# liuruiyang98/Jittor-MLP

Measured on AMD Instinct MI355X. Metric: images/sec fwd, 224^2 bs=256/GPU, Mixer-B/16, higher is better.
Workload: dtype bf16

## Files before the change

### jittor-mlp_amd/csrc/gen/t4emu.py

```python
import os
import struct
import sys

import numpy as np

sys.path.insert(0, os.path.dirname(os.path.abspath(__file__)))
import isa
import t4gen
from q4emu import from16, gelu_ref, to16

S_TOK, KPAD = 196, 224


def w2_slot_source():
    slot = np.arange(32)
    kk, h, e = slot >> 4, (slot >> 3) & 1, slot & 7
    return 16 * kk + 8 * (e >> 2) + 4 * h + (e & 3)


def pack(w1, b1, w2, b2, dt, dt2=None):
    T, S = w1.shape
    G = (T + 31) // 32
    w1p = np.zeros((G * 32, 256), np.uint16)
    w1p[:T, :S] = to16(w1, dt)
# ... 25 lines not shown
        q = f16(c[0] * u + c[1]).astype(np.float64)
        for k in range(2, 7):
            q = f16(q * u + c[k]).astype(np.float64)
        p = np.clip(f16(t * q + 0.5).astype(np.float64), 0.0, 1.0)
        return f16(h * p).astype(np.float64)


def plan(M, t_rows, G, grid, nimg):
    tpi = t_rows // 256
    nit = G + 2
    lead = nit & 1
    return dict(M=M, G=G, ldxt=KPAD, ldx=t_rows, ntiles=M // 256, tpi=tpi, tpi_magic=(((1 << 31) + tpi - 1) // tpi) & 0xFFFFFFFF,
                grid=grid, stat_ld=nimg * S_TOK * 2, nit=nit + lead, lead=lead, S=S_TOK)


class T4Emu(isa.Emu):
    def __init__(self, gen, mem, karg_addr, bid, **kw):
        asm = isa.Asm()
        asm.ins = list(gen.a.ins)
        super().__init__(asm, mem, lds_bytes=163840, nwaves=4, **kw)
        self.karg_addr, self.bid = karg_addr, bid

    def init(self, waves):
        for w in waves:
            w.s[0] = self.karg_addr & 0xFFFFFFFF
            w.s[1] = self.karg_addr >> 32
            w.s[2] = self.bid
            w.v[0] = (np.arange(64) + 64 * w.wid).astype(np.uint32)
            w.v[1:] = 0x7FC0BEEF
            w.a[:] = 0x7FC0BEEF
        self.lds[:] = 0xEE


def run_case(gen, nimg=1, t_rows=512, T=80, grid=1, seed=0, dma_mode="late", order=None, verbose=False):
    rng = np.random.default_rng(seed)
    dt = gen.dtype
    S = S_TOK
    M = nimg * t_rows
    xt = np.zeros((M, KPAD), np.uint16)
    xt[:, :S] = to16(rng.uniform(-1, 1, (M, S)), dt)
    w1 = rng.uniform(-1, 1, (T, S)) * 0.15
    b1 = rng.uniform(-1, 1, T).astype(np.float32)
    w2 = rng.uniform(-1, 1, (S, T)) * 0.2
    b2 = rng.uniform(-1, 1, S).astype(np.float32)
    x0 = to16(rng.uniform(-2, 2, (nimg * S, t_rows)), dt)
    ln = getattr(gen, "ln", False)
    if ln:
        gamma = rng.uniform(0.5, 1.5, t_rows).astype(np.float32)
        beta = rng.uniform(-0.5, 0.5, t_rows).astype(np.float32)
        xf = from16(x0, dt).astype(np.float64)
        mean = xf.mean(axis=1).astype(np.float32)
        rstd = (1.0 / np.sqrt(xf.var(axis=1) + 1e-5)).astype(np.float32)
        xn = ((xf - mean[:, None].astype(np.float64)) * rstd[:, None].astype(np.float64)) * gamma[None, :] + beta[None, :]
        xt[:, :S] = to16(xn.reshape(nimg, S, t_rows).transpose(0, 2, 1).reshape(M, S), dt)
    dt2 = "f16" if getattr(gen, "h2", False) else dt
    w1p, b1p, w2p, b2p, G = pack(w1, b1, w2, b2, dt, dt2)
    mem = isa.Mem()
    aXt, aW1, aW2, aB1, aB2 = mem.add(xt), mem.add(w1p), mem.add(w2p), mem.add(b1p), mem.add(b2p)
    aX = mem.add(x0, writable=True)
    nplanes = t_rows // 64
    stats = np.full((nplanes, nimg * S, 2), np.nan, np.float32)
    aSt = mem.add(stats, writable=True)
    pl = plan(M, t_rows, G, grid, nimg)
    ka = bytearray(t4gen.ARG_BYTES)
    for name, val in (("xt", aXt), ("w1", aW1), ("w2", aW2), ("b1", aB1), ("b2", aB2), ("x", aX), ("stats", aSt), ("prof", 0)):
        struct.pack_into("<Q", ka, t4gen.KA[name], val)
    for name, val in pl.items():
        struct.pack_into("<I", ka, t4gen.KA[name], val)
    if ln:
        for name, arr in (("ln_mean", mean), ("ln_rstd", rstd), ("gamma", gamma), ("beta", beta)):
            struct.pack_into("<Q", ka, t4gen.KA[name], mem.add(arr))
        struct.pack_into("<Q", ka, t4gen.KA["xt"], 0)
    karg = mem.add(np.frombuffer(bytes(ka), np.uint8))
    nins = 0
    for bid in range(grid):
        e = T4Emu(gen, mem, karg, bid, dma_mode=dma_mode, order=order)
        waves = e.run()
        nins += sum(w.nissued for w in waves)
    out = from16(mem.get(aX).view(np.uint16).reshape(nimg * S, t_rows), dt).astype(np.float64)
    X = from16(xt[:, :S], dt).astype(np.float64)
    W1 = from16(to16(w1, dt), dt).astype(np.float64)
    W2 = from16(to16(w2, dt2), dt2).astype(np.float64)
    hid = gelu_ref(X @ W1.T + b1[None, :].astype(np.float64))
    hid = from16(to16(hid, dt2), dt2).astype(np.float64)
    y = hid @ W2.T + b2[None, :].astype(np.float64)
    y = y.reshape(nimg, t_rows, S).transpose(0, 2, 1).reshape(nimg * S, t_rows)
    ref = from16(to16(y + from16(x0, dt).astype(np.float64), dt), dt).astype(np.float64)
    err = np.abs(out - ref)
    tol = (2.0 ** -7 * 2.0 if dt == "bf16" else 2.0 ** -10 * 1.5) * np.maximum(1.0, np.abs(ref))
    bad = ~(err <= tol)
    ok = not bad.any()
    if getattr(gen, "h2", False):
        pre = (X @ W1.T).astype(np.float32) + b1[None, :]
        y2 = h2_gelu_ref(pre) @ W2.T + b2[None, :].astype(np.float64)
        y2 = y2.reshape(nimg, t_rows, S).transpose(0, 2, 1).reshape(nimg * S, t_rows)
        ref2 = from16(to16(y2 + from16(x0, dt).astype(np.float64), dt), dt).astype(np.float64)
        d2 = np.abs(out - ref2)
        ulp = 2.0 ** (np.floor(np.log2(np.maximum(np.abs(ref2), 0.5))) - 7)
        frac = float((d2 > 0).mean())
        if verbose:
            print("  against the operation-by-operation restatement of the packed-f16 GELU: %.2f %% of the outputs differ, max %.2f ulp" %
                  (100 * frac, float((d2 / ulp).max())))
        if not ((d2 <= ulp).all() and frac < 0.03):
            print("  FAILED the restatement check: %.2f %% differ, max %.2f ulp" % (100 * frac, float((d2 / ulp).max())))
            ok = False
    if verbose or bad.any():
        print("case nimg=%d t_rows=%d T=%d (G=%d) grid=%d mode=%s: bad %d of %d, max err %.3g, instructions %d" %
              (nimg, t_rows, T, G, grid, dma_mode, bad.sum(), bad.size, np.nanmax(err) if np.isfinite(err).any() else float("nan"), nins))
        if bad.any():
            idx = np.argwhere(bad)
            print("  first bad (token row, channel):", idx[:8].tolist())
# ... 23 lines not shown
```

### jittor-mlp_amd/csrc/gen/t4gen.py

```python
import os
import sys

sys.path.insert(0, os.path.dirname(os.path.abspath(__file__)))
from isa import A, F, S, V, Asm, Neg, Reg, h2bits
from q4gen import GELU, GELU_FORM, GELU_H2, GELU_RAW, GELU_SIG, SQRT2, Alloc, h2_gelu_ops, h2b_gelu_ops, sig_gelu_ops

KA = dict(xt=0, w1=8, w2=16, b1=24, b2=32, x=40, stats=48, prof=56,
          M=64, G=68, ldxt=72, ldx=76, ntiles=80, tpi=84, tpi_magic=88, grid=92, stat_ld=96, nit=100, lead=104, S=108,
          ln_mean=112, ln_rstd=120, gamma=128, beta=136)
ARG_BYTES = 144
LN_WAVE = 2 * 8 * 272

W1_PITCH, W1_PIECES = 528, 17
W2_PITCH, W2_PIECES = 80, 18
W1_STAGE, W2_STAGE = W1_PIECES * 1024, W2_PIECES * 1024
W1_OFF, W2_OFF = 0, 2 * W1_STAGE
B1_OFF = W2_OFF + 2 * W2_STAGE
STG_PITCH = 272
STG_WAVE = 32 * STG_PITCH
STG_OFF = B1_OFF + 4096
STG_BUF = 4 * STG_WAVE
LDS_BYTES = STG_OFF + 2 * STG_BUF
W2_GROUP_BYTES = 224 * 64
W1_MAGIC, W2_MAGIC = 1986, 13108
assert all((o * W1_MAGIC) >> 20 == o // W1_PITCH for o in range(0, W1_STAGE, 16))
assert all((o * W2_MAGIC) >> 20 == o // W2_PITCH for o in range(0, W2_STAGE, 16))


class T4:
    NKS, NTB = 13, 7
    NXA = 8
    DEPTH = 3

    def __init__(self, dtype="bf16", stats=False, dbg=0, name=None, shape=0, ln=False, h2=False):
        assert not ln or shape
        self.ln = ln
        self.shape = shape
        self.dtype, self.stats, self.dbg = dtype, stats, dbg
        assert not h2 or dtype == "bf16"
        self.h2 = h2
        self.name = name or "t4_%s%s%s%s" % (dtype, "_h2" if h2 else "", "_st" if stats else "", ("", "_odd", "_even")[shape] + ("_ln" if ln else ""))
        self.mfma = "v_mfma_f32_32x32x16_bf16" if dtype == "bf16" else "v_mfma_f32_32x32x16_f16"
        self.mfma2 = "v_mfma_f32_32x32x16_f16" if h2 else self.mfma
        self.cvt = "v_cvt_pk_bf16_f32" if dtype == "bf16" else "v_cvt_pk_f16_f32"
        self.dot = "v_dot2c_f32_bf16" if dtype == "bf16" else "v_dot2c_f32_f16"
        self.raw = GELU_RAW[dtype]
        self.coefs = GELU[dtype][1]
        self.a = Asm()
        self.build()

    def regs(self):
        s = Alloc("s", 33, 100)
        v = Alloc("v", 1, 256)
        self.s_karg, self.s_bid, self.v_tid = S(0, 2), S(2), V(0)
        self.p = {k: S(4 + 2 * i, 2) for i, k in enumerate(["xt", "w1", "w2", "b1", "b2", "x", "stats", "prof"])}
        self.k = {k: S(20 + i) for i, k in enumerate(["M", "G", "ldxt", "ldx", "ntiles", "tpi", "tpi_magic", "grid", "stat_ld", "nit", "lead", "S"])}
        self.s_wave, self.s_tile, self.s_next, self.s_has = s("wave"), s("tile"), s("next"), s("has")
        self.s_g, self.s_cnt = s("g"), s("cnt")
        self.s_wv1k, self.s_w2x = s("wv1k"), s("w2x")
        self.s_w1src, self.s_w2src = s("w1src", 2, 2), s("w2src", 2, 2)
        self.s_xb = [s("xb%d" % rb, 2, 2) for rb in range(2)]
        self.s_ocur, self.s_lcur = s("ocur", 2, 2), s("lcur", 2, 2)
        self.s_scur = s("scur", 2, 2) if self.stats else None
        self.s_tok8 = s("tok8")
        self.s_r2 = s("r2")
        self.sig = GELU_FORM[self.dtype] == "sig" and not self.h2
        self.h2b = GELU_FORM[self.dtype] == "h2b" and not self.h2
        self.s_k0, self.s_k1 = (s("gk0"), s("gk1")) if (self.sig or self.h2b) else (None, None)
        self.s_hscale, self.s_hc6 = (s("hscale"), s("hc6")) if self.h2 else (None, None)
        self.s_mask = s("mask", 2, 2)
        self.s_t = [s("t%d" % i) for i in range(6)]
        self.s_t64 = s("t64", 2, 2)
        self.s_prof0 = s("prof0", 2, 2)
        self.s_prof1, self.s_epi = s("prof1", 2, 2), s("epi")
        self.s_ph = [s("ph%d" % i) for i in range(3)]
        if self.ln:
            self.s_lnp = s("lnp", 8, 4)
            self.s_lx, self.s_lmean, self.s_lrstd = s("lx", 2, 2), s("lmean", 2, 2), s("lrstd", 2, 2)
            self.s_l16 = s("l16")
        self.ns = s.next
        self.X = [[None] * self.NKS for _ in range(2)]
        na = 0
        for rb in range(2):
            for ks in range(self.NKS):
                if rb == 1 and ks >= self.NKS - self.NXA:
                    self.X[rb][ks] = A(224 + 4 * na, 4)
                    na += 1
                else:
                    self.X[rb][ks] = v("X%d_%d" % (rb, ks), 4, 2)
        self.Wf = [v("Wf%d" % b, 4, 2) for b in range(4)]
        self.b1 = v("b1", 16, 2)
        self.xg = [[v("xg%d_%d" % (par, rb), 16, 2) for rb in range(2)] for par in range(2)]
        self.h = [[[v("h%d_%d_%d" % (par, rb, kk), 4, 2) for kk in range(2)] for rb in range(2)] for par in range(2)]
        self.tmp = [[v("g%s%d" % (n, ch), 2, 2) for n in "tuq"] for ch in range(2)]
        flat = [r_[e] for grp_ in self.tmp for r_ in grp_ for e in range(2)]
        self.tmp_t, self.tmp_u, self.tmp_q = flat[0:4], flat[4:8], flat[8:12]
        self.v_c0 = v("c0")
        self.v_hc = [v("hc%d" % j) for j in range(1, 6)] if (self.h2 or self.h2b) else None
        self.v_hp = [v("hp%d" % j) for j in range(2)] if self.h2b else None
        self.v_nz = v("negzero") if self.h2b else None
        self.v_w1rd, self.v_w2rd, self.v_b1rd = v("w1rd"), v("w2rd"), v("b1rd")
        self.v_w1off = [v("w1off%d" % i) for i in range(5)]
        self.v_w2off = [v("w2off%d" % i) for i in range(5)]
        self.v_xoff = v("xoff")
        self.v_stw, self.v_strd, self.v_ooff = v("stw"), v("strd"), v("ooff")
        self.v_soff = v("soff") if self.stats else None
        self.v_b2 = [v("b2_%d" % tb) for tb in range(self.NTB)]
        self.nv = v.next
# ... 200 lines not shown
            self.wait_lds(rd[n])
            wf = self.Wf[n & 3]
            for rb in range(2):
                if kind == "w2":
                    mfma(self.D2(rb, tb), self.h[par][rb][x], wf, self.D2(rb, tb), op=self.mfma2)
                else:
                    mfma(self.xg[par][rb], wf, self.X[rb][x], self.b1 if x == 0 else self.xg[par][rb])
        while state["done"] < total:
            fill[state["done"]]()
            state["done"] += 1
        while xl:
            emit_xload()
        assert not dma
        a("s_add_i32", self.s_g, self.s_g, 1)
        a("v_add_u32", self.v_b1rd, 128, self.v_b1rd)

    def tile_xbase(self, tile):
        a, t, k = self.a, self.s_t, self.k
        a("s_lshl_b32", t[0], tile, 8)
        a("s_lshl_b32", t[1], self.s_wave, 6)
        a("s_add_u32", t[0], t[0], t[1])
        self.mul64(self.s_t64, t[0], k["ldxt"], 1)
        self.add64(self.s_xb[0], self.p["xt"], self.s_t64[0], self.s_t64[1])
        a("s_lshl_b32", t[0], k["ldxt"], 6)
        self.add64(self.s_xb[1], self.s_xb[0], t[0])

    def x_loads(self):
        if self.dbg & 32:
            return
        for rb in range(2):
            for ks in range(self.NKS):
                self.vload("global_load_dwordx4", self.X[rb][ks], self.v_xoff, self.s_xb[rb], offset=32 * ks)

    def ln_loader(self, tile):
        a, t, k, p = self.a, self.s_t, self.k, self.p
        bf = self.dtype == "bf16"
        xg = self.xg
        ldr = [[xg[0][0][0:4], xg[0][0][4:8], xg[0][0][8:10], xg[0][0][10:12]],
               [xg[0][1][0:4], xg[0][1][4:8], xg[0][1][8:10], xg[0][1][10:12]]]
        gam, bet = [xg[1][0][e] for e in range(8)], [xg[1][0][8 + e] for e in range(8)]
        fa, fb = [xg[1][1][e] for e in range(8)], [xg[1][1][8 + e] for e in range(8)]
        hb = self.h[0][0][0].idx
        pk = [Reg("v", hb + e) for e in range(8)]
        lane, pp, c8, va0, va1, vst, vgb, vw = [Reg("v", hb + 8 + i) for i in range(8)]
        vr = [Reg("v", hb + 16), Reg("v", hb + 17)]
        x1, x2, mneg = Reg("v", hb + 18), Reg("v", hb + 19), [Reg("v", hb + 20), Reg("v", hb + 21)]
        a("s_lshl_b32", t[0], tile, 1)
        a("s_mul_hi_u32", t[1], t[0], k["tpi_magic"])
        a("s_mul_i32", t[0], t[1], k["tpi"])
        a("s_sub_u32", t[0], tile, t[0])
        a("s_lshl_b32", t[0], t[0], 8)
        a("s_lshl_b32", t[2], self.s_wave, 6)
        a("s_add_u32", t[2], t[2], t[0])
        a("s_mul_i32", t[3], t[1], k["S"])
        self.mul64(self.s_t64, t[3], k["ldx"], 1)
        a("s_lshl_b32", t[0], t[2], 1)
        self.add64(self.s_t64, self.s_t64, t[0])
        self.add64(self.s_lx, p["x"], self.s_t64[0], self.s_t64[1])
        a("s_lshl_b32", t[0], t[3], 2)
        self.add64(self.s_lmean, self.s_lnp[0:2], t[0])
        self.add64(self.s_lrstd, self.s_lnp[2:4], t[0])
        a("s_lshl_b32", t[0], t[2], 2)
        self.add64(self.s_t64, self.s_lnp[4:6], t[0])
        a("s_lshl_b32", self.s_l16, k["ldx"], 5)
        a("v_and_b32", lane, 63, self.v_tid)
        a("v_lshrrev_b32", pp, 3, lane)
        a("v_and_b32", c8, 7, lane)
        a("v_lshlrev_b32", vgb, 5, c8)
        a("global_load_dwordx4", Reg("v", gam[0].idx, 4), vgb, self.s_t64)
        a("global_load_dwordx4", Reg("v", gam[4].idx, 4), vgb, self.s_t64, offset=16)
        self.add64(self.s_t64, self.s_lnp[6:8], t[0])
        a("v_mul_lo_u32", x1, pp, k["ldx"])
        a("v_lshlrev_b32", x1, 2, x1)
        a("v_lshl_add_u32", va0, c8, 4, x1)
        a("s_lshl_b32", t[0], k["ldx"], 1)
        a("v_add_u32", va1, t[0], va0)
        a("v_lshlrev_b32", vst, 3, pp)
        a("global_load_dwordx4", Reg("v", bet[0].idx, 4), vgb, self.s_t64)
        a("global_load_dwordx4", Reg("v", bet[4].idx, 4), vgb, self.s_t64, offset=16)
        a("s_mul_i32", t[0], self.s_wave, LN_WAVE)
        a("s_add_u32", t[0], t[0], STG_OFF)
        a("v_lshl_add_u32", x1, c8, 3, pp)
        a("v_lshl_add_u32", vw, x1, 2, t[0])
        a("v_and_b32", x1, 31, lane)
        a("v_lshrrev_b32", x2, 5, lane)
        for rb in range(2):
            a("v_and_b32", vr[rb], 7, x1)
            a("v_mul_u32_u24", vr[rb], 272, vr[rb])
            a("v_lshrrev_b32", mneg[0], 3, x1)
            a("v_add_u32", mneg[0], 4 * rb, mneg[0])
            a("v_lshl_add_u32", mneg[0], mneg[0], 1, x2)
            a("v_lshl_add_u32", vr[rb], mneg[0], 4, vr[rb])
            a("v_add_u32", vr[rb], t[0], vr[rb])
        nks = self.NKS

        def loads(ks):
            buf = ldr[ks & 1]
            last = ks == nks - 1
            if last:
                a("s_mov_b32", self.s_t64[0], 0xFFFF)
                a("s_mov_b32", self.s_t64[1], 0)
                a("s_mov_b64", "exec", self.s_t64)
            a("global_load_dwordx4", buf[0], va0, self.s_lx)
            a("global_load_dwordx4", buf[1], va1, self.s_lx)
            a("global_load_dwordx2", buf[2], vst, self.s_lmean)
            a("global_load_dwordx2", buf[3], vst, self.s_lrstd)
            if last:
                a("s_mov_b64", "exec", -1)
            else:
                self.add64(self.s_lx, self.s_lx, self.s_l16)
                self.add64(self.s_lmean, self.s_lmean, 64)
                self.add64(self.s_lrstd, self.s_lrstd, 64)
        loads(0)
        for ks in range(nks):
            if ks + 1 < nks:
                loads(ks + 1)
            a("s_waitcnt", vmcnt=4 if ks + 1 < nks else 0)
            buf = ldr[ks & 1]
            for tok, f in ((0, fa), (1, fb)):
                q = buf[tok]
                for d in range(4):
                    if bf:
                        a("v_lshlrev_b32", f[2 * d], 16, q[d])
                        a("v_and_b32", f[2 * d + 1], 0xFFFF0000, q[d])
                    else:
                        a("v_lshrrev_b32", f[2 * d + 1], 16, q[d])
                        a("v_cvt_f32_f16", f[2 * d], q[d])
                        a("v_cvt_f32_f16", f[2 * d + 1], f[2 * d + 1])
                a("v_mul_f32", mneg[tok], Neg(buf[2][tok]), buf[3][tok])
            for tok, f in ((0, fa), (1, fb)):
                for e in range(8):
                    a("v_fma_f32", f[e], f[e], buf[3][tok], mneg[tok])
            for tok, f in ((0, fa), (1, fb)):
                for e in range(8):
                    a("v_fma_f32", f[e], f[e], gam[e], bet[e])
            for e in range(8):
                a(self.cvt, pk[e], fa[e], fb[e])
            for e in range(8):
                a("ds_write_b32", vw, pk[e], offset=(ks & 1) * 8 * 272 + e * 272)
            for rb in range(2):
                a("ds_read_b128", self.X[rb][ks], vr[rb], offset=(ks & 1) * 8 * 272)
        a("s_waitcnt", lgkmcnt=0)

    def tile_scalars(self):
        a, t, k, p = self.a, self.s_t, self.k, self.p
        a("s_lshl_b32", t[0], self.s_tile, 1)
        a("s_mul_hi_u32", t[1], t[0], k["tpi_magic"])
        a("s_mul_i32", t[0], t[1], k["tpi"])
        a("s_sub_u32", t[0], self.s_tile, t[0])
        a("s_lshl_b32", t[0], t[0], 8)
        a("s_lshl_b32", t[2], self.s_wave, 6)
        a("s_add_u32", t[2], t[2], t[0])
        a("s_mul_i32", t[3], t[1], k["S"])
        self.mul64(self.s_t64, t[3], k["ldx"], 1)
        a("s_lshl_b32", t[0], t[2], 1)
        self.add64(self.s_t64, self.s_t64, t[0])
        self.add64(self.s_ocur, p["x"], self.s_t64[0], self.s_t64[1])
        a("s_mov_b32", self.s_lcur[0], self.s_ocur[0])
        a("s_mov_b32", self.s_lcur[1], self.s_ocur[1])
        if self.stats:
            a("s_lshr_b32", t[0], t[2], 6)
            self.mul64(self.s_t64, t[0], k["stat_ld"], 2)
            a("s_lshl_b32", t[0], t[3], 3)
            self.add64(self.s_t64, self.s_t64, t[0])
            self.add64(self.s_scur, p["stats"], self.s_t64[0], self.s_t64[1])

    def res_loads(self, tb):
        a = self.a
        rec = []
        rounds = 4 if tb < self.NTB - 1 else 1
        if rounds == 1:
            a("s_mov_b64", "exec", self.s_mask)
        for r in range(rounds):
            if self.dbg & 16:
# ... 39 lines not shown
                        a("v_and_b32", self.e_t[1], 0xFFFF0000, rr[c])
                    else:
                        a("v_lshrrev_b32", self.e_t[1], 16, rr[c])
                        a("v_cvt_f32_f16", self.e_t[0], rr[c])
                        a("v_cvt_f32_f16", self.e_t[1], self.e_t[1])
                    a("v_pk_add_f32", pin, pin, self.e_t)
                    a(self.cvt, rr[c], pin[0], pin[1])
                if self.stats:
                    sp = self.e_sp
                    a("v_mov_b32", sp[0], 0)
                    a("v_mov_b32", sp[1], 0)
                    for c in range(4):
                        a(self.dot, sp[0], rr[c], self.e_ones)
                        a(self.dot, sp[1], rr[c], rr[c])
                    for n_, mod in enumerate((dict(quad_perm="[1,0,3,2]"), dict(quad_perm="[2,3,0,1]"), dict(row_half_mirror=True))):
                        a("s_nop", 1 if n_ == 0 else 0)
                        a("v_add_f32_dpp", sp[0], sp[0], sp[0], **mod, row_mask="0xf", bank_mask="0xf")
                        a("v_add_f32_dpp", sp[1], sp[1], sp[1], **mod, row_mask="0xf", bank_mask="0xf")
                    a("s_mov_b32", self.s_t64[0], 0x01010101)
                    a("s_mov_b32", self.s_t64[1], 0x01010101 if rounds == 4 else 0)
                    a("s_mov_b64", "exec", self.s_t64)
                    a("global_store_dwordx2", self.v_soff, sp, self.s_scur)
                    a("s_mov_b64", "exec", -1)
                    self.add64(self.s_scur, self.s_scur, 64)
                if not (self.dbg & 4):
                    if rounds == 1:
                        a("s_mov_b64", "exec", self.s_mask)
                    a("global_store_dwordx4", self.v_ooff, rr, self.s_ocur)
                    if rounds == 1:
                        a("s_mov_b64", "exec", -1)
                self.add64(self.s_ocur, self.s_ocur, self.s_tok8)
            if tb + 2 < self.NTB:
                res[tb + 2] = self.res_loads(tb + 2)

    def build(self):
        a = self.a
        self.regs()
        self.lgkm_issued = 0
        self.vm_loads = 0
        t, k, p = self.s_t, self.k, self.p
        L_end, L_tile, L_iter, L_nonext = a.newlabel("END"), a.newlabel("TILE"), a.newlabel("ITER"), a.newlabel("NONEXT")
        a("s_load_dwordx16", S(4, 16), self.s_karg, 0)
        a("s_load_dwordx8", S(20, 8), self.s_karg, 64)
        a("s_load_dwordx4", S(28, 4), self.s_karg, 96)
        if self.ln:
            a("s_load_dwordx4", self.s_lnp[0:4], self.s_karg, KA["ln_mean"])
            a("s_load_dwordx4", self.s_lnp[4:8], self.s_karg, KA["gamma"])
        lane, j, h, l3, l7, x, y, z = (self.tmp[0][0][0], self.tmp[0][0][1], self.tmp[0][1][0], self.tmp[0][1][1], self.tmp[0][2][0],
                                       self.tmp[0][2][1], self.tmp[1][0][0], self.tmp[1][0][1])
        a("v_and_b32", lane, 63, self.v_tid)
        a("v_lshrrev_b32", x, 6, self.v_tid)
        a("s_nop", 0)
        a("v_readfirstlane_b32", self.s_wave, x)
        a("v_and_b32", j, 31, lane)
        a("v_lshrrev_b32", h, 5, lane)
        a("v_lshrrev_b32", l3, 3, lane)
        a("v_and_b32", l7, 7, lane)
        a("s_mov_b32", self.s_r2, F(SQRT2))
        if self.h2:
            a("v_mov_b32", self.v_c0, h2bits(GELU_H2["coefs"][0]))
            a("s_mov_b32", self.s_hscale, h2bits(GELU_H2["scale"]))
            for cj in range(5):
                a("v_mov_b32", self.v_hc[cj], h2bits(GELU_H2["coefs"][cj + 1]))
            a("s_mov_b32", self.s_hc6, h2bits(GELU_H2["coefs"][6]))
        elif self.h2b:
            a("v_mov_b32", self.v_c0, h2bits(GELU_H2["coefs"][0]))
# ... 49 lines not shown
        a("s_add_u32", t[0], t[0], STG_OFF)
        a("v_mul_u32_u24", x, STG_PITCH, j)
        a("v_lshl_add_u32", x, h, 4, x)
        a("v_add_u32", self.v_stw, t[0], x)
        a("v_mul_u32_u24", x, STG_PITCH, l3)
        a("v_lshl_add_u32", x, l7, 5, x)
        a("v_add_u32", self.v_strd, t[0], x)
        a("v_mul_lo_u32", x, l3, k["ldx"])
        a("v_lshlrev_b32", x, 1, x)
        a("v_lshl_add_u32", self.v_ooff, l7, 4, x)
        if self.stats:
            a("v_lshlrev_b32", self.v_soff, 3, l3)
        a("s_lshl_b32", self.s_tok8, k["ldx"], 4)
        a("v_lshlrev_b32", x, 4, self.v_tid)
        a("global_load_dwordx4", self.e_acc[0], x, p["b1"])
        a("s_mov_b32", self.s_tile, self.s_bid)
        a("s_cmp_ge_u32", self.s_tile, k["ntiles"])
        a("v_add_u32", x, B1_OFF, x)
        a("s_waitcnt", vmcnt=0)
        a("ds_write_b128", x, self.e_acc[0])
        a("s_cbranch_scc1", L_end)
        a("v_lshlrev_b32", y, 2, j)
        for tb in range(self.NTB):
            a("global_load_dword", self.v_b2[tb], y, p["b2"], offset=128 * tb)
        a("s_sub_u32", t[0], 0, k["lead"])
        self.dma_sources()
        if not (self.dbg & 1):
            for i in range(5):
                for kind in ("w1", "w2"):
                    self.emit_m0(kind, i, 0)
                    a("s_nop", 0)
                    self.emit_dma(kind, i, 0)
        if self.ln:
            self.ln_loader(self.s_tile)
        else:
            self.tile_xbase(self.s_tile)
            self.x_loads()
        a("s_sub_u32", t[0], 2, k["lead"])
        a("s_lshl_b32", t[0], t[0], 7)
        a("v_add_u32", self.v_b1rd, t[0], self.v_b1rd)
        a("s_waitcnt", vmcnt=0 if ((self.dbg & 33) or self.ln) else 10 + 2 * self.NKS)
        a.label(L_tile)
        self.tile_scalars()
        for rb in range(2):
            for tb in range(self.NTB):
                for r in range(16):
                    a("v_accvgpr_write_b32", A(16 * (self.NTB * rb + tb) + r), self.v_b2[tb])
        if self.shape == 0:
            for par in range(2):
                for rb in range(2):
                    for r in range(16):
                        a("v_mov_b32", self.xg[par][rb][r], 0)
                    for kk in range(2):
                        for r in range(4):
                            a("v_mov_b32", self.h[par][rb][kk][r], 0)
        a("s_sub_u32", self.s_g, 0, k["lead"])
        nx = 0 if ((self.dbg & 32) or self.ln) else 2 * self.NKS
        xl_on = not self.ln
        if self.shape == 0:
            a("s_lshr_b32", self.s_cnt, k["nit"], 1)
            a.label(L_iter)
            self.iteration(0)
            self.iteration(1)
            a("s_sub_u32", self.s_cnt, self.s_cnt, 1)
            a("s_cmp_lg_u32", self.s_cnt, 0)
            a("s_cbranch_scc1", L_iter)
        else:
            L_skip = a.newlabel("NOLOOP")

            def stamp(acc):
                a("s_memtime", self.s_t64)
                a("s_waitcnt", lgkmcnt=0)
                a("s_sub_u32", t[0], self.s_t64[0], self.s_prof1[0])
                a("s_add_u32", acc, acc, t[0])
                a("s_mov_b32", self.s_prof1[0], self.s_t64[0])
            a("s_memtime", self.s_prof1)
            a("s_waitcnt", lgkmcnt=0)
            if self.shape == 1:
                self.iteration(0, fc2=False, fc1=False, gelu=False)
                self.iteration(1, fc2=False, gelu=False)
                self.iteration(0, fc2=False)
                first, second = 1, 0
                a("s_sub_u32", self.s_cnt, k["G"], 3)
            else:
                self.iteration(0, fc2=False, gelu=False)
                self.iteration(1, fc2=False)
                first, second = 0, 1
                a("s_sub_u32", self.s_cnt, k["G"], 2)
            stamp(self.s_ph[0])
            a("s_lshr_b32", self.s_cnt, self.s_cnt, 1)
            a("s_cmp_eq_u32", self.s_cnt, 0)
            a("s_cbranch_scc1", L_skip)
            a.label(L_iter)
            self.iteration(first)
            self.iteration(second)
            a("s_sub_u32", self.s_cnt, self.s_cnt, 1)
            a("s_cmp_lg_u32", self.s_cnt, 0)
            a("s_cbranch_scc1", L_iter)
            a.label(L_skip)
            if self.shape == 1:
                self.iteration(1)
                stamp(self.s_ph[1])
                self.iteration(0, fc1=False, xload=xl_on)
                self.iteration(1, fc1=False, gelu=False, vm_allow=nx)
            else:
                stamp(self.s_ph[1])
                self.iteration(0, fc1=False, xload=xl_on)
                self.iteration(1, fc1=False, gelu=False, vm_allow=nx)
            stamp(self.s_ph[2])
        a("s_lshl_b32", t[0], k["nit"], 7)
        a("v_sub_u32", self.v_b1rd, self.v_b1rd, t[0])
        if self.ln:
            a("s_add_u32", self.s_next, self.s_tile, k["grid"])
            a("s_cmp_lt_u32", self.s_next, k["ntiles"])
            a("s_cselect_b32", self.s_has, 1, 0)
        if self.shape == 0:
            a("s_add_u32", self.s_next, self.s_tile, k["grid"])
            a("s_cmp_lt_u32", self.s_next, k["ntiles"])
            a("s_cselect_b32", self.s_has, 1, 0)
            a("s_cbranch_scc0", L_nonext)
            self.tile_xbase(self.s_next)
            self.x_loads()
            a.label(L_nonext)
        self.lgkm_issued = 0
        self.vm_loads = 0
        a("s_memtime", self.s_prof1)
        a("s_nop", 7)
        a("s_nop", 7)
        res = {0: self.res_loads(0), 1: self.res_loads(1)}
        self.epilogue(res)
        a("s_memtime", self.s_t64)
        a("s_waitcnt", lgkmcnt=0)
        a("s_sub_u32", t[0], self.s_t64[0], self.s_prof1[0])
        a("s_add_u32", self.s_epi, self.s_epi, t[0])
        a("s_mov_b32", self.s_tile, self.s_next)
        a("s_cmp_lg_u32", self.s_has, 0)
        if self.ln:
            a("s_cbranch_scc0", L_end)
            self.ln_loader(self.s_tile)
            a("s_branch", L_tile)
        else:
            a("s_cbranch_scc1", L_tile)
        a.label(L_end)
        L_noprof = a.newlabel("NOPROF")
        a("s_memtime", self.s_t64)
        a("s_or_b32", t[0], p["prof"][0], p["prof"][1])
        a("s_cmp_eq_u32", t[0], 0)
        a("s_cbranch_scc1", L_noprof)
        a("s_waitcnt", lgkmcnt=0)
        a("s_sub_u32", self.s_t64[0], self.s_t64[0], self.s_prof0[0])
        a("s_lshl_b32", t[0], self.s_bid, 5)
        a("v_mov_b32", self.e_sp[0], t[0])
        a("v_mov_b32", self.e_t[0], self.s_t64[0])
        a("v_mov_b32", self.e_t[1], self.s_epi)
        a("global_store_dwordx2", self.e_sp[0], self.e_t, p["prof"])
        a("s_nop", 1)
        a("v_mov_b32", self.e_t[0], self.s_ph[0])
        a("v_mov_b32", self.e_t[1], self.s_ph[1])
        a("global_store_dwordx2", self.e_sp[0], self.e_t, p["prof"], offset=8)
        a("s_nop", 1)
        a("v_mov_b32", self.e_t[0], self.s_ph[2])
        a("global_store_dword", self.e_sp[0], self.e_t[0], p["prof"], offset=16)
        a.label(L_noprof)
        a("s_waitcnt", vmcnt=0, lgkmcnt=0)
        a("s_endpgm")


def variants():
    out = []
    for dt in ("bf16", "f16"):
        for st in (False, True):
            for shape in (0, 1, 2):
                out.append(dict(dtype=dt, stats=st, shape=shape))
            for shape in (1, 2):
                out.append(dict(dtype=dt, stats=st, shape=shape, ln=True))
    for st in (False, True):
        for shape in (0, 1, 2):
            out.append(dict(dtype="bf16", stats=st, shape=shape, h2=True))
        for shape in (1, 2):
            out.append(dict(dtype="bf16", stats=st, shape=shape, ln=True, h2=True))
    for dbg in (1, 2, 4, 3, 16, 32, 48, 52):
        out.append(dict(dtype="bf16", stats=True, dbg=dbg, name="t4_bf16_st_dbg%d" % dbg))
    return out


def kernel_text(gen):
    assert gen.nv <= 248, "the compiler needs a few VGPRs of its own (the thread id operand, WWM)"
    clob = ['"v%d"' % i for i in range(gen.nv)] + ['"a%d"' % i for i in range(256)] + ['"s%d"' % i for i in range(gen.ns) if i != 32] + ['"vcc"', '"memory"']
    body = ['"s_mov_b64 s[0:1], %0\\n\\t"', '"s_mov_b32 s2, %1\\n\\t"', '"v_mov_b32 v0, %2\\n\\t"', gen.a.c_string()]
    return ("extern \"C\" __global__ void __launch_bounds__(256, 1) %s(const mlpk::T4Args args) {\n"
            "    asm volatile(\n%s\n        :\n        : \"s\"(__builtin_amdgcn_kernarg_segment_ptr()), \"s\"(blockIdx.x), \"v\"(threadIdx.x)\n"
            "        : %s);\n}\n" % (gen.name, "\n".join(body), ", ".join(clob)))


def emit(path):
    import isa
    out = ["// GENERATED by csrc/gen/t4gen.py -- do not edit.  One asm block per kernel: every register is named by the generator.\n"]
    table = []
    for kw in variants():
        g = T4(**kw)
        pr = isa.lint(g.a)
        if pr:
            raise RuntimeError("%s: %d hazard lint findings, first: %s" % (g.name, len(pr), pr[0]))
        out.append(kernel_text(g))
        table.append((g.name, kw))
    out.append("namespace mlpk {\nstruct T4Variant { const char* name; const void* fn; int dtype, stats, dbg, shape, ln, h2; };\n"
               "static const T4Variant kT4Variants[] = {\n")
    for name, kw in table:
        out.append("    {\"%s\", reinterpret_cast<const void*>(&%s), %s, %d, %d, %d, %d, %d},\n" %
                   (name, name, "MLPK_BF16" if kw["dtype"] == "bf16" else "MLPK_F16", kw["stats"], kw.get("dbg", 0), kw.get("shape", 0), kw.get("ln", False),
                    kw.get("h2", False)))
    out.append("};\n}  // namespace mlpk\n")
    text = "".join(out)
    if not os.path.exists(path) or open(path).read() != text:
        with open(path, "w") as f:
            f.write(text)
    return len(table)


if __name__ == "__main__":
    if len(sys.argv) > 1:
        print("wrote %d kernels to %s" % (emit(sys.argv[1]), sys.argv[1]))
    else:
        import isa
        g = T4(stats=True)
        print("instructions:", len(g.a.ins), "vgprs:", g.nv, "sgprs:", g.ns)
        isa.lint(g.a, verbose=True)
```

### jittor-mlp_amd/csrc/mlpk_tokenmlp_t4.hip

```cpp
#include "mlpk_common.h"
#include "mlpk_tokenmlp_t4.h"
#include <cstdlib>

namespace mlpk {
struct T4Args {
    const void* xt;
    const void* w1;
    const void* w2;
    const float* b1;
    const float* b2;
    void* x;
    float* stats;
    void* prof;
    int M, G, ldxt, ldx;
    int ntiles, tpi, tpi_magic, grid;
    int stat_ld, nit, lead, S;
    const float* ln_mean;
    const float* ln_rstd;
    const float* gamma;
    const float* beta;
};
static_assert(sizeof(T4Args) == 144, "kernarg layout");
}

#include "gen_out/t4_kernels.inc"

namespace mlpk {

#define T4_LDS_BYTES 145408

static int t4_grid_cap() {
    static int cap = 0;
    if (!cap) {
        int dev = 0, cu = 0;
        if (hipGetDevice(&dev) != hipSuccess || hipDeviceGetAttribute(&cu, hipDeviceAttributeMultiprocessorCount, dev) != hipSuccess || cu < 1) cu = 256;
        cap = cu;
    }
    return cap;
}

bool t4_supported(int dtype, int S, int G, int ldxt, int M, int t_rows, int ldx) {
    if (dtype != MLPK_BF16 && dtype != MLPK_F16) return false;
    if (S != 196 || ldxt != 224) return false;
    if (G < 1 || G > 28) return false;
    if (t_rows <= 0 || t_rows % 256 || M <= 0 || M % t_rows) return false;
    if (ldx % 8 || ldx < t_rows) return false;
    return true;
}

int t4_launch(const T4Call& c, hipStream_t stream) {
    if (!t4_supported(c.dtype, c.S, c.G, c.ldxt, c.M, c.t_rows, c.ldx)) return MLPK_ESHAPE;
    int shape = (c.G & 1) ? (c.G >= 3 ? 1 : 0) : (c.G >= 2 ? 2 : 0);
    const char* es = getenv("MLPK_T4_SHAPE");
    if (c.dbg || (es && es[0] == '0')) shape = 0;
    const int ln = c.ln_mean != nullptr;
    if (c.h2 && (c.dtype != MLPK_BF16 || c.dbg)) return MLPK_EMODE;
    if (ln && (!shape || !c.ln_rstd || !c.gamma || !c.beta)) return MLPK_ESHAPE;
    const T4Variant* v = nullptr;
    for (const T4Variant& k : kT4Variants)
        if (k.dtype == c.dtype && k.stats == (c.stats != nullptr) && k.dbg == c.dbg && k.shape == shape && k.ln == ln && k.h2 == c.h2) { v = &k; break; }
    if (!v) return MLPK_ESHAPE;
    T4Args a;
    a.xt = c.xt; a.w1 = c.w1; a.w2 = c.w2; a.b1 = c.b1; a.b2 = c.b2; a.x = c.x; a.stats = c.stats; a.prof = c.prof;
    a.M = c.M; a.G = c.G; a.ldxt = c.ldxt; a.ldx = c.ldx;
    a.ntiles = c.M / 256;
    a.tpi = c.t_rows / 256;
    a.tpi_magic = (int)(((1ull << 31) + a.tpi - 1) / a.tpi);
    a.grid = a.ntiles < t4_grid_cap() ? a.ntiles : t4_grid_cap();
    a.stat_ld = (c.M / c.t_rows) * c.S * 2;
    a.lead = (c.G + 2) & 1;
    a.nit = c.G + 2 + a.lead;
    a.S = c.S;
    a.ln_mean = c.ln_mean; a.ln_rstd = c.ln_rstd; a.gamma = c.gamma; a.beta = c.beta;
    hipError_t e = hipFuncSetAttribute(v->fn, hipFuncAttributeMaxDynamicSharedMemorySize, T4_LDS_BYTES);
    if (e != hipSuccess) return (int)e;
    void* params[] = {&a};
    e = hipLaunchKernel(v->fn, dim3(a.grid), dim3(256), params, T4_LDS_BYTES, stream);
    if (e != hipSuccess) return (int)e;
    MLPK_LAUNCH_CHECK();
    return 0;
}

}
```

Before: 36760.

## Prefetch next tile's LayerNorm inputs during epilogue in token-MLP kernel

Adds a scheduled variant of the fused-LayerNorm token-MLP kernel. It issues the next tile's gamma/beta and first K-step input loads before the epilogue, reusing freed weight and hidden registers as a four-deep buffer ring. It also moves the LN staging area to its own LDS region so it no longer aliases the store staging buffers. The goal is to hide the global-load latency of the LN loader behind the epilogue. The cost is more LDS per block and more register-lifetime coupling, and the variant is selected by default whenever LN is fused. Adds a profiling stamp for the LN phase.

Measured after the change: 36860 (median of 6 runs). Within noise of the previous version (+0.3%).

```diff
diff --git a/jittor-mlp_amd/csrc/gen/t4emu.py b/jittor-mlp_amd/csrc/gen/t4emu.py
--- a/jittor-mlp_amd/csrc/gen/t4emu.py
+++ b/jittor-mlp_amd/csrc/gen/t4emu.py
@@ -81,7 +81,7 @@
         self.lds[:] = 0xEE
 
 
-def run_case(gen, nimg=1, t_rows=512, T=80, grid=1, seed=0, dma_mode="late", order=None, verbose=False):
+def run_case(gen, nimg=1, t_rows=512, T=80, grid=1, seed=0, dma_mode="late", order=None, verbose=False, outputs=None):
     rng = np.random.default_rng(seed)
     dt = gen.dtype
     S = S_TOK
@@ -126,6 +126,9 @@
         e = T4Emu(gen, mem, karg, bid, dma_mode=dma_mode, order=order)
         waves = e.run()
         nins += sum(w.nissued for w in waves)
+    if outputs is not None:
+        outputs["x"] = mem.get(aX).view(np.uint16).copy()
+        outputs["stats"] = mem.get(aSt).view(np.uint32).copy()
     out = from16(mem.get(aX).view(np.uint16).reshape(nimg * S, t_rows), dt).astype(np.float64)
     X = from16(xt[:, :S], dt).astype(np.float64)
     W1 = from16(to16(w1, dt), dt).astype(np.float64)
diff --git a/jittor-mlp_amd/csrc/gen/t4gen.py b/jittor-mlp_amd/csrc/gen/t4gen.py
--- a/jittor-mlp_amd/csrc/gen/t4gen.py
+++ b/jittor-mlp_amd/csrc/gen/t4gen.py
@@ -20,7 +20,8 @@
 STG_WAVE = 32 * STG_PITCH
 STG_OFF = B1_OFF + 4096
 STG_BUF = 4 * STG_WAVE
-LDS_BYTES = STG_OFF + 2 * STG_BUF
+LN_OFF = STG_OFF + 2 * STG_BUF
+LDS_BYTES = LN_OFF + 4 * LN_WAVE
 W2_GROUP_BYTES = 224 * 64
 W1_MAGIC, W2_MAGIC = 1986, 13108
 assert all((o * W1_MAGIC) >> 20 == o // W1_PITCH for o in range(0, W1_STAGE, 16))
@@ -32,14 +33,16 @@
     NXA = 8
     DEPTH = 3
 
-    def __init__(self, dtype="bf16", stats=False, dbg=0, name=None, shape=0, ln=False, h2=False):
+    def __init__(self, dtype="bf16", stats=False, dbg=0, name=None, shape=0, ln=False, h2=False, sched=0):
         assert not ln or shape
         self.ln = ln
+        assert not sched or ln
+        self.sched = sched
         self.shape = shape
         self.dtype, self.stats, self.dbg = dtype, stats, dbg
         assert not h2 or dtype == "bf16"
         self.h2 = h2
-        self.name = name or "t4_%s%s%s%s" % (dtype, "_h2" if h2 else "", "_st" if stats else "", ("", "_odd", "_even")[shape] + ("_ln" if ln else ""))
+        self.name = name or "t4_%s%s%s%s" % (dtype, "_h2" if h2 else "", "_st" if stats else "", ("", "_odd", "_even")[shape] + ("_ln" if ln else "") + ("_pf" if sched else ""))
         self.mfma = "v_mfma_f32_32x32x16_bf16" if dtype == "bf16" else "v_mfma_f32_32x32x16_f16"
         self.mfma2 = "v_mfma_f32_32x32x16_f16" if h2 else self.mfma
         self.cvt = "v_cvt_pk_bf16_f32" if dtype == "bf16" else "v_cvt_pk_f16_f32"
@@ -73,7 +76,7 @@
         self.s_t64 = s("t64", 2, 2)
         self.s_prof0 = s("prof0", 2, 2)
         self.s_prof1, self.s_epi = s("prof1", 2, 2), s("epi")
-        self.s_ph = [s("ph%d" % i) for i in range(3)]
+        self.s_ph = [s("ph%d" % i) for i in range(4)]
         if self.ln:
             self.s_lnp = s("lnp", 8, 4)
             self.s_lx, self.s_lmean, self.s_lrstd = s("lx", 2, 2), s("lmean", 2, 2), s("lrstd", 2, 2)
@@ -340,19 +343,8 @@
             for ks in range(self.NKS):
                 self.vload("global_load_dwordx4", self.X[rb][ks], self.v_xoff, self.s_xb[rb], offset=32 * ks)
 
-    def ln_loader(self, tile):
+    def ln_tile_scalars(self, tile):
         a, t, k, p = self.a, self.s_t, self.k, self.p
-        bf = self.dtype == "bf16"
-        xg = self.xg
-        ldr = [[xg[0][0][0:4], xg[0][0][4:8], xg[0][0][8:10], xg[0][0][10:12]],
-               [xg[0][1][0:4], xg[0][1][4:8], xg[0][1][8:10], xg[0][1][10:12]]]
-        gam, bet = [xg[1][0][e] for e in range(8)], [xg[1][0][8 + e] for e in range(8)]
-        fa, fb = [xg[1][1][e] for e in range(8)], [xg[1][1][8 + e] for e in range(8)]
-        hb = self.h[0][0][0].idx
-        pk = [Reg("v", hb + e) for e in range(8)]
-        lane, pp, c8, va0, va1, vst, vgb, vw = [Reg("v", hb + 8 + i) for i in range(8)]
-        vr = [Reg("v", hb + 16), Reg("v", hb + 17)]
-        x1, x2, mneg = Reg("v", hb + 18), Reg("v", hb + 19), [Reg("v", hb + 20), Reg("v", hb + 21)]
         a("s_lshl_b32", t[0], tile, 1)
         a("s_mul_hi_u32", t[1], t[0], k["tpi_magic"])
         a("s_mul_i32", t[0], t[1], k["tpi"])
@@ -371,6 +363,81 @@
         a("s_lshl_b32", t[0], t[2], 2)
         self.add64(self.s_t64, self.s_lnp[4:6], t[0])
         a("s_lshl_b32", self.s_l16, k["ldx"], 5)
+
+    def ln_lds_addresses(self, lane, x1, x2, mneg, vw, vr, pp, c8):
+        a, t = self.a, self.s_t
+        a("s_mul_i32", t[0], self.s_wave, LN_WAVE)
+        a("s_add_u32", t[0], t[0], LN_OFF)
+        a("v_lshl_add_u32", x1, c8, 3, pp)
+        a("v_lshl_add_u32", vw, x1, 2, t[0])
+        a("v_and_b32", x1, 31, lane)
+        a("v_lshrrev_b32", x2, 5, lane)
+        for rb in range(2):
+            a("v_and_b32", vr[rb], 7, x1)
+            a("v_mul_u32_u24", vr[rb], 272, vr[rb])
+            a("v_lshrrev_b32", mneg[0], 3, x1)
+            a("v_add_u32", mneg[0], 4 * rb, mneg[0])
+            a("v_lshl_add_u32", mneg[0], mneg[0], 1, x2)
+            a("v_lshl_add_u32", vr[rb], mneg[0], 4, vr[rb])
+            a("v_add_u32", vr[rb], t[0], vr[rb])
+
+    def ln_kloads(self, ks, buf, va0, va1, vst):
+        a = self.a
+        last = ks == self.NKS - 1
+        if last:
+            a("s_mov_b32", self.s_t64[0], 0xFFFF)
+            a("s_mov_b32", self.s_t64[1], 0)
+            a("s_mov_b64", "exec", self.s_t64)
+        a("global_load_dwordx4", buf[0], va0, self.s_lx)
+        a("global_load_dwordx4", buf[1], va1, self.s_lx)
+        a("global_load_dwordx2", buf[2], vst, self.s_lmean)
+        a("global_load_dwordx2", buf[3], vst, self.s_lrstd)
+        if last:
+            a("s_mov_b64", "exec", -1)
+        else:
+            self.add64(self.s_lx, self.s_lx, self.s_l16)
+            self.add64(self.s_lmean, self.s_lmean, 64)
+            self.add64(self.s_lrstd, self.s_lrstd, 64)
+
+    def ln_kstep(self, ks, buf, gam, bet, fa, fb, pk, mneg, vw, vr):
+        a = self.a
+        for tok, f in ((0, fa), (1, fb)):
+            q = buf[tok]
+            for d in range(4):
+                if self.dtype == "bf16":
+                    a("v_lshlrev_b32", f[2 * d], 16, q[d])
+                    a("v_and_b32", f[2 * d + 1], 0xFFFF0000, q[d])
+                else:
+                    a("v_lshrrev_b32", f[2 * d + 1], 16, q[d])
+                    a("v_cvt_f32_f16", f[2 * d], q[d])
+                    a("v_cvt_f32_f16", f[2 * d + 1], f[2 * d + 1])
+            a("v_mul_f32", mneg[tok], Neg(buf[2][tok]), buf[3][tok])
+        for tok, f in ((0, fa), (1, fb)):
+            for e in range(8):
+                a("v_fma_f32", f[e], f[e], buf[3][tok], mneg[tok])
+        for tok, f in ((0, fa), (1, fb)):
+            for e in range(8):
+                a("v_fma_f32", f[e], f[e], gam[e], bet[e])
+        for e in range(8):
+            a(self.cvt, pk[e], fa[e], fb[e])
+        for e in range(8):
+            a("ds_write_b32", vw, pk[e], offset=(ks & 1) * 8 * 272 + e * 272)
+        for rb in range(2):
+            a("ds_read_b128", self.X[rb][ks], vr[rb], offset=(ks & 1) * 8 * 272)
+
+    def ln_loader(self, tile):
+        a, t, k = self.a, self.s_t, self.k
+        xg = self.xg
+        ldr = [[xg[0][0][0:4], xg[0][0][4:8], xg[0][0][8:10], xg[0][0][10:12]],
+               [xg[0][1][0:4], xg[0][1][4:8], xg[0][1][8:10], xg[0][1][10:12]]]
+        gam, bet = [xg[1][0][e] for e in range(8)], [xg[1][0][8 + e] for e in range(8)]
+        fa, fb = [xg[1][1][e] for e in range(8)], [xg[1][1][8 + e] for e in range(8)]
+        hb = self.h[0][0][0].idx
+        pk = [Reg("v", hb + e) for e in range(8)]
+        lane, pp, c8, va0, va1, vst, vgb, vw = [Reg("v", hb + 8 + i) for i in range(8)]
+        vr = [Reg("v", hb + 16), Reg("v", hb + 17)]
+        x1, x2, mneg = Reg("v", hb + 18), Reg("v", hb + 19), [Reg("v", hb + 20), Reg("v", hb + 21)]
+        self.ln_tile_scalars(tile)
         a("v_and_b32", lane, 63, self.v_tid)
         a("v_lshrrev_b32", pp, 3, lane)
         a("v_and_b32", c8, 7, lane)
@@ -386,68 +453,75 @@
         a("v_lshlrev_b32", vst, 3, pp)
         a("global_load_dwordx4", Reg("v", bet[0].idx, 4), vgb, self.s_t64)
         a("global_load_dwordx4", Reg("v", bet[4].idx, 4), vgb, self.s_t64, offset=16)
-        a("s_mul_i32", t[0], self.s_wave, LN_WAVE)
-        a("s_add_u32", t[0], t[0], STG_OFF)
-        a("v_lshl_add_u32", x1, c8, 3, pp)
-        a("v_lshl_add_u32", vw, x1, 2, t[0])
-        a("v_and_b32", x1, 31, lane)
-        a("v_lshrrev_b32", x2, 5, lane)
-        for rb in range(2):
-            a("v_and_b32", vr[rb], 7, x1)
-            a("v_mul_u32_u24", vr[rb], 272, vr[rb])
-            a("v_lshrrev_b32", mneg[0], 3, x1)
-            a("v_add_u32", mneg[0], 4 * rb, mneg[0])
-            a("v_lshl_add_u32", mneg[0], mneg[0], 1, x2)
-            a("v_lshl_add_u32", vr[rb], mneg[0], 4, vr[rb])
-            a("v_add_u32", vr[rb], t[0], vr[rb])
+        self.ln_lds_addresses(lane, x1, x2, mneg, vw, vr, pp, c8)
         nks = self.NKS
-
-        def loads(ks):
-            buf = ldr[ks & 1]
-            last = ks == nks - 1
-            if last:
-                a("s_mov_b32", self.s_t64[0], 0xFFFF)
-                a("s_mov_b32", self.s_t64[1], 0)
-                a("s_mov_b64", "exec", self.s_t64)
-            a("global_load_dwordx4", buf[0], va0, self.s_lx)
-            a("global_load_dwordx4", buf[1], va1, self.s_lx)
-            a("global_load_dwordx2", buf[2], vst, self.s_lmean)
-            a("global_load_dwordx2", buf[3], vst, self.s_lrstd)
-            if last:
-                a("s_mov_b64", "exec", -1)
-            else:
-                self.add64(self.s_lx, self.s_lx, self.s_l16)
-                self.add64(self.s_lmean, self.s_lmean, 64)
-                self.add64(self.s_lrstd, self.s_lrstd, 64)
-        loads(0)
+        self.ln_kloads(0, ldr[0], va0, va1, vst)
         for ks in range(nks):
             if ks + 1 < nks:
-                loads(ks + 1)
+                self.ln_kloads(ks + 1, ldr[(ks + 1) & 1], va0, va1, vst)
             a("s_waitcnt", vmcnt=4 if ks + 1 < nks else 0)
-            buf = ldr[ks & 1]
-            for tok, f in ((0, fa), (1, fb)):
-                q = buf[tok]
-                for d in range(4):
-                    if bf:
-                        a("v_lshlrev_b32", f[2 * d], 16, q[d])
-                        a("v_and_b32", f[2 * d + 1], 0xFFFF0000, q[d])
-                    else:
-                        a("v_lshrrev_b32", f[2 * d + 1], 16, q[d])
-                        a("v_cvt_f32_f16", f[2 * d], q[d])
-                        a("v_cvt_f32_f16", f[2 * d + 1], f[2 * d + 1])
-                a("v_mul_f32", mneg[tok], Neg(buf[2][tok]), buf[3][tok])
-            for tok, f in ((0, fa), (1, fb)):
-                for e in range(8):
-                    a("v_fma_f32", f[e], f[e], buf[3][tok], mneg[tok])
-            for tok, f in ((0, fa), (1, fb)):
-                for e in range(8):
-                    a("v_fma_f32", f[e], f[e], gam[e], bet[e])
-            for e in range(8):
-                a(self.cvt, pk[e], fa[e], fb[e])
-            for e in range(8):
-                a("ds_write_b32", vw, pk[e], offset=(ks & 1) * 8 * 272 + e * 272)
-            for rb in range(2):
-                a("ds_read_b128", self.X[rb][ks], vr[rb], offset=(ks & 1) * 8 * 272)
+            self.ln_kstep(ks, ldr[ks & 1], gam, bet, fa, fb, pk, mneg, vw, vr)
+        a("s_waitcnt", lgkmcnt=0)
+
+    LN_PRE, LN_AHEAD = 2, 3
+
+    def ln_regs_pf(self):
+        xg, h, wf = self.xg, self.h, self.Wf
+        quads = lambda q0, q1, q2: [q0, q1, q2[0:2], q2[2:4]]
+        bufs = [quads(wf[0], wf[1], wf[2]), quads(h[1][0][0], h[1][0][1], h[1][1][0]),
+                [xg[0][0][0:4], xg[0][0][4:8], xg[0][0][8:10], xg[0][0][10:12]], [xg[0][1][0:4], xg[0][1][4:8], xg[0][1][8:10], xg[0][1][10:12]]]
+        gam, bet = [self.b1[e] for e in range(8)], [self.b1[8 + e] for e in range(8)]
+        va0, va1, vst = self.tmp[1][0][0], self.tmp[1][0][1], self.tmp[1][1][0]
+        return bufs, gam, bet, va0, va1, vst
+
+    def ln_prefetch(self, tile):
+        a, t, k = self.a, self.s_t, self.k
+        bufs, gam, bet, va0, va1, vst = self.ln_regs_pf()
+        lane, pp, c8, vgb = [self.Wf[3][i] for i in range(4)]
+        x1 = self.h[1][1][1][0]
+        self.ln_tile_scalars(tile)
+        a("v_and_b32", lane, 63, self.v_tid)
+        a("v_lshrrev_b32", pp, 3, lane)
+        a("v_and_b32", c8, 7, lane)
+        a("v_lshlrev_b32", vgb, 5, c8)
+        a("global_load_dwordx4", Reg("v", gam[0].idx, 4), vgb, self.s_t64)
+        a("global_load_dwordx4", Reg("v", gam[4].idx, 4), vgb, self.s_t64, offset=16)
+        self.add64(self.s_t64, self.s_lnp[6:8], t[0])
+        a("v_mul_lo_u32", x1, pp, k["ldx"])
+        a("v_lshlrev_b32", x1, 2, x1)
+        a("v_lshl_add_u32", va0, c8, 4, x1)
+        a("s_lshl_b32", t[0], k["ldx"], 1)
+        a("v_add_u32", va1, t[0], va0)
+        a("v_lshlrev_b32", vst, 3, pp)
+        a("global_load_dwordx4", Reg("v", bet[0].idx, 4), vgb, self.s_t64)
+        a("global_load_dwordx4", Reg("v", bet[4].idx, 4), vgb, self.s_t64, offset=16)
+        for ks in range(self.LN_PRE):
+            self.ln_kloads(ks, bufs[ks], va0, va1, vst)
+
+    def ln_loader_pf(self):
+        a = self.a
+        bufs, gam, bet, va0, va1, vst = self.ln_regs_pf()
+        nb = self.LN_AHEAD + 1
+        assert nb == len(bufs) and self.LN_PRE <= self.LN_AHEAD
+        xg = self.xg
+        fa, fb = [xg[1][1][e] for e in range(8)], [xg[1][1][8 + e] for e in range(8)]
+        pk = [xg[1][0][e] for e in range(8)]
+        hb = self.h[0][0][0].idx
+        lane, pp, c8, vw, x1, x2 = [Reg("v", hb + i) for i in range(6)]
+        vr = [Reg("v", hb + 6), Reg("v", hb + 7)]
+        mneg = [Reg("v", hb + 8), Reg("v", hb + 9)]
+        a("v_and_b32", lane, 63, self.v_tid)
+        a("v_lshrrev_b32", pp, 3, lane)
+        a("v_and_b32", c8, 7, lane)
+        self.ln_lds_addresses(lane, x1, x2, mneg, vw, vr, pp, c8)
+        nks = self.NKS
+        issued = self.LN_PRE
+        for ks in range(nks):
+            while issued < min(ks + 1 + self.LN_AHEAD, nks):
+                self.ln_kloads(issued, bufs[issued % nb], va0, va1, vst)
+                issued += 1
+            a("s_waitcnt", vmcnt=4 * (issued - ks - 1))
+            self.ln_kstep(ks, bufs[ks % nb], gam, bet, fa, fb, pk, mneg, vw, vr)
         a("s_waitcnt", lgkmcnt=0)
 
     def tile_scalars(self):
@@ -553,6 +627,23 @@
                 self.add64(self.s_ocur, self.s_ocur, self.s_tok8)
             if tb + 2 < self.NTB:
                 res[tb + 2] = self.res_loads(tb + 2)
+
+    def stamp(self, acc):
+        a, t = self.a, self.s_t
+        a("s_memtime", self.s_t64)
+        a("s_waitcnt", lgkmcnt=0)
+        a("s_sub_u32", t[0], self.s_t64[0], self.s_prof1[0])
+        a("s_add_u32", acc, acc, t[0])
+        a("s_mov_b32", self.s_prof1[0], self.s_t64[0])
+
+    def timed_ln_loader(self, tile):
+        self.a("s_memtime", self.s_prof1)
+        self.a("s_waitcnt", lgkmcnt=0)
+        if self.sched:
+            self.ln_loader_pf()
+        else:
+            self.ln_loader(tile)
+        self.stamp(self.s_ph[3])
 
     def build(self):
         a = self.a
@@ -668,7 +759,9 @@
                     a("s_nop", 0)
                     self.emit_dma(kind, i, 0)
         if self.ln:
-            self.ln_loader(self.s_tile)
+            if self.sched:
+                self.ln_prefetch(self.s_tile)
+            self.timed_ln_loader(self.s_tile)
         else:
             self.tile_xbase(self.s_tile)
             self.x_loads()
@@ -704,12 +797,7 @@
         else:
             L_skip = a.newlabel("NOLOOP")
 
-            def stamp(acc):
-                a("s_memtime", self.s_t64)
-                a("s_waitcnt", lgkmcnt=0)
-                a("s_sub_u32", t[0], self.s_t64[0], self.s_prof1[0])
-                a("s_add_u32", acc, acc, t[0])
-                a("s_mov_b32", self.s_prof1[0], self.s_t64[0])
+            stamp = self.stamp
             a("s_memtime", self.s_prof1)
             a("s_waitcnt", lgkmcnt=0)
             if self.shape == 1:
@@ -764,6 +852,11 @@
         a("s_nop", 7)
         a("s_nop", 7)
         res = {0: self.res_loads(0), 1: self.res_loads(1)}
+        if self.sched:
+            a("s_cmp_lt_u32", self.s_next, k["ntiles"])
+            a("s_cselect_b32", t[4], self.s_next, self.s_tile)
+            self.ln_prefetch(t[4])
+            self.vm_loads += 4 + 4 * self.LN_PRE
         self.epilogue(res)
         a("s_memtime", self.s_t64)
         a("s_waitcnt", lgkmcnt=0)
@@ -773,7 +866,7 @@
         a("s_cmp_lg_u32", self.s_has, 0)
         if self.ln:
             a("s_cbranch_scc0", L_end)
-            self.ln_loader(self.s_tile)
+            self.timed_ln_loader(self.s_tile)
             a("s_branch", L_tile)
         else:
             a("s_cbranch_scc1", L_tile)
@@ -796,7 +889,8 @@
         a("global_store_dwordx2", self.e_sp[0], self.e_t, p["prof"], offset=8)
         a("s_nop", 1)
         a("v_mov_b32", self.e_t[0], self.s_ph[2])
-        a("global_store_dword", self.e_sp[0], self.e_t[0], p["prof"], offset=16)
+        a("v_mov_b32", self.e_t[1], self.s_ph[3])
+        a("global_store_dwordx2", self.e_sp[0], self.e_t, p["prof"], offset=16)
         a.label(L_noprof)
         a("s_waitcnt", vmcnt=0, lgkmcnt=0)
         a("s_endpgm")
@@ -809,12 +903,14 @@
             for shape in (0, 1, 2):
                 out.append(dict(dtype=dt, stats=st, shape=shape))
             for shape in (1, 2):
-                out.append(dict(dtype=dt, stats=st, shape=shape, ln=True))
+                for sched in (0, 1):
+                    out.append(dict(dtype=dt, stats=st, shape=shape, ln=True, sched=sched))
     for st in (False, True):
         for shape in (0, 1, 2):
             out.append(dict(dtype="bf16", stats=st, shape=shape, h2=True))
         for shape in (1, 2):
-            out.append(dict(dtype="bf16", stats=st, shape=shape, ln=True, h2=True))
+            for sched in (0, 1):
+                out.append(dict(dtype="bf16", stats=st, shape=shape, ln=True, h2=True, sched=sched))
     for dbg in (1, 2, 4, 3, 16, 32, 48, 52):
         out.append(dict(dtype="bf16", stats=True, dbg=dbg, name="t4_bf16_st_dbg%d" % dbg))
     return out
@@ -840,12 +936,12 @@
             raise RuntimeError("%s: %d hazard lint findings, first: %s" % (g.name, len(pr), pr[0]))
         out.append(kernel_text(g))
         table.append((g.name, kw))
-    out.append("namespace mlpk {\nstruct T4Variant { const char* name; const void* fn; int dtype, stats, dbg, shape, ln, h2; };\n"
+    out.append("namespace mlpk {\nstruct T4Variant { const char* name; const void* fn; int dtype, stats, dbg, shape, ln, h2, sched; };\n"
                "static const T4Variant kT4Variants[] = {\n")
     for name, kw in table:
-        out.append("    {\"%s\", reinterpret_cast<const void*>(&%s), %s, %d, %d, %d, %d, %d},\n" %
+        out.append("    {\"%s\", reinterpret_cast<const void*>(&%s), %s, %d, %d, %d, %d, %d, %d},\n" %
                    (name, name, "MLPK_BF16" if kw["dtype"] == "bf16" else "MLPK_F16", kw["stats"], kw.get("dbg", 0), kw.get("shape", 0), kw.get("ln", False),
-                    kw.get("h2", False)))
+                    kw.get("h2", False), kw.get("sched", 0)))
     out.append("};\n}  // namespace mlpk\n")
     text = "".join(out)
     if not os.path.exists(path) or open(path).read() != text:
diff --git a/jittor-mlp_amd/csrc/mlpk_tokenmlp_t4.hip b/jittor-mlp_amd/csrc/mlpk_tokenmlp_t4.hip
--- a/jittor-mlp_amd/csrc/mlpk_tokenmlp_t4.hip
+++ b/jittor-mlp_amd/csrc/mlpk_tokenmlp_t4.hip
@@ -27,7 +27,7 @@
 
 namespace mlpk {
 
-#define T4_LDS_BYTES 145408
+#define T4_LDS_BYTES 162816
 
 static int t4_grid_cap() {
     static int cap = 0;
@@ -56,9 +56,12 @@
     const int ln = c.ln_mean != nullptr;
     if (c.h2 && (c.dtype != MLPK_BF16 || c.dbg)) return MLPK_EMODE;
     if (ln && (!shape || !c.ln_rstd || !c.gamma || !c.beta)) return MLPK_ESHAPE;
+    const char* ss = getenv("MLPK_T4_SCHED");
+    const int sched = (ln && !(ss && ss[0] == '0')) ? 1 : 0;
     const T4Variant* v = nullptr;
     for (const T4Variant& k : kT4Variants)
-        if (k.dtype == c.dtype && k.stats == (c.stats != nullptr) && k.dbg == c.dbg && k.shape == shape && k.ln == ln && k.h2 == c.h2) { v = &k; break; }
+        if (k.dtype == c.dtype && k.stats == (c.stats != nullptr) && k.dbg == c.dbg && k.shape == shape && k.ln == ln && k.h2 == c.h2 &&
+            k.sched == sched) { v = &k; break; }
     if (!v) return MLPK_ESHAPE;
     T4Args a;
     a.xt = c.xt; a.w1 = c.w1; a.w2 = c.w2; a.b1 = c.b1; a.b2 = c.b2; a.x = c.x; a.stats = c.stats; a.prof = c.prof;
```
